# Jan-Celin/SCCG-genome-compression

Hardware: AMD Instinct MI355X
Metric: target bases compressed/sec at 1/2/4/8 GPUs; bit-exact record stream vs CPU ref (higher is better)
Workload: dtype u8

## Files before the change

### sccg-genome-compression_amd/csrc/ingest.hip

```cpp
#include "internal.h"

namespace {

constexpr int PER_T = INGEST_TILE / SCCG_BLOCK;
constexpr int WPB = SCCG_BLOCK / 64;


constexpr int64_t FM_CHUNK = 16384;
template <int NW>
__device__ __forceinline__ uint8_t wb(const uint32_t (&w)[NW], int i) { return (uint8_t)(w[i >> 2] >> (8 * (i & 3))); }
template <int NW>
__device__ __forceinline__ void load_words(const uint8_t* __restrict__ buf, int64_t n, int64_t off, uint32_t (&w)[NW]);
__global__ __launch_bounds__(SCCG_BLOCK) void k_first_match(const uint8_t* __restrict__ buf, int64_t n,
                                                            const int64_t* __restrict__ from_slot, int mode, uint8_t c,
                                                            int64_t* __restrict__ res, unsigned int* __restrict__ ticket) {
    __shared__ int64_t s_cs;
    const int64_t from = from_slot ? *from_slot + 1 : 0;
    const int64_t base = from & ~(int64_t)63;
    constexpr int PER = FM_CHUNK / SCCG_BLOCK;
    for (;;) {
        if (threadIdx.x == 0) {
            const int64_t cs = base + (int64_t)atomicAdd(ticket, 1u) * FM_CHUNK;
            const int64_t best = (int64_t)__hip_atomic_load((unsigned long long*)res, __ATOMIC_RELAXED, __HIP_MEMORY_SCOPE_AGENT);
            s_cs = (cs >= n || cs >= best) ? -1 : cs;
// ... 663 lines not shown
            if (q >= 0 && t - q > RUNS_LOOKBACK) atomicOr(ovf, 2);
            const uint32_t first = (uint32_t)(f >> 1) & 3u;
#pragma unroll
            for (int p = 0; p < 2; p++) {
                const uint32_t fp = (first >> p) & 1u, pp = (prev >> p) & 1u;
                if (fp && !pp) b |= 1 << (2 * p);
                if (!fp && pp) b |= 2 << (2 * p);
            }
        }
        bev[t] = b;
        cs[t] = (int64_t)((c & 0xffff) + (b & 1)) | ((int64_t)(((c >> 32) & 0xffff) + ((b >> 2) & 1)) << 32);
        ce[t] = (int64_t)(((c >> 16) & 0xffff) + ((b >> 1) & 1)) | ((int64_t)((c >> 48) + ((b >> 3) & 1)) << 32);
    }
}

__global__ void k_runs_copy(int64_t ntiles, const int64_t* __restrict__ toff, const uint64_t* __restrict__ rc,
                            const int32_t* __restrict__ bev, const int64_t* __restrict__ cs, const int64_t* __restrict__ ce,
                            RunSlots rsl, int32_t* __restrict__ rs_l, int32_t* __restrict__ re_l,
                            int32_t* __restrict__ rs_n, int32_t* __restrict__ re_n) {
    for (int64_t t = (int64_t)blockIdx.x * blockDim.x + threadIdx.x; t < ntiles; t += (int64_t)gridDim.x * blockDim.x) {
        const uint64_t c = rc[t];
        const int32_t b = bev[t];
        const int32_t t0 = (int32_t)toff[t];
        const size_t sb = (size_t)t * RUN_SLOT;
        int32_t* const dst[4] = {rs_l, re_l, rs_n, re_n};
        const int32_t* const src[4] = {rsl.sl, rsl.el, rsl.sn, rsl.en};
        const int64_t base[4] = {cs[t] & 0xffffffff, ce[t] & 0xffffffff, cs[t] >> 32, ce[t] >> 32};
#pragma unroll
        for (int q = 0; q < 4; q++) {
            const int end = q & 1;
            int64_t at = base[q];
            if ((b >> q) & 1) dst[q][at++] = t0 - end;
            const int nq = (int)((c >> (16 * q)) & 0xffff);
            for (int k = 0; k < nq && k < RUN_SLOT; k++) dst[q][at++] = src[q][sb + k] - end;
        }
    }
}

__global__ void k_runs_fin(const int64_t* __restrict__ tot, const int64_t* __restrict__ d_nT, int32_t* __restrict__ re_l,
                           int32_t* __restrict__ re_n, int64_t* __restrict__ d_nruns) {
    const int64_t sl = tot[0] & 0xffffffff, sn = tot[0] >> 32, el = tot[1] & 0xffffffff, en = tot[1] >> 32;
    if (sl > el) re_l[sl - 1] = (int32_t)(*d_nT - 1);
    if (sn > en) re_n[sn - 1] = (int32_t)(*d_nT - 1);
    d_nruns[0] = sl;
    d_nruns[1] = sn;
}

__device__ __forceinline__ int64_t run_text_len(int32_t d, int32_t len, bool at_end) {
    return len == 1 ? (int64_t)ndigits_i32(d) + (at_end ? 0 : 1) : (int64_t)(3 + ndigits_i32(d) + ndigits_i32(len));
}

__global__ void k_run_textlen(const int32_t* __restrict__ rs, const int32_t* __restrict__ re, int64_t nr,
                              int64_t n, int64_t* __restrict__ len) {
    for (int64_t r = (int64_t)blockIdx.x * blockDim.x + threadIdx.x; r < nr; r += (int64_t)gridDim.x * blockDim.x) {
        const int32_t d = rs[r] - (r ? rs[r - 1] : 0);
        len[r] = run_text_len(d, re[r] - rs[r] + 1, (int64_t)re[r] == n - 1);
    }
}

__global__ void k_run_textwrite(const int32_t* __restrict__ rs, const int32_t* __restrict__ re, int64_t nr,
                                int64_t n, const int64_t* __restrict__ off, uint8_t* __restrict__ out) {
    for (int64_t r = (int64_t)blockIdx.x * blockDim.x + threadIdx.x; r < nr; r += (int64_t)gridDim.x * blockDim.x) {
        const int32_t d = rs[r] - (r ? rs[r - 1] : 0);
        const int32_t len = re[r] - rs[r] + 1;
        uint8_t* o = out + off[r];
        if (len == 1) {
            o += write_i32(o, d);
            if ((int64_t)re[r] != n - 1) *o = ',';
        } else {
            *o++ = '(';
            o += write_i32(o, d);
            *o++ = ',';
            o += write_i32(o, len);
            *o = ')';
        }
    }
}

}

constexpr int FH_T = 256, FH_PER = 64;
__global__ __launch_bounds__(FH_T) void k_find_header(const uint8_t* __restrict__ buf, int64_t n, int64_t* __restrict__ d_sc,
                                                      int32_t* __restrict__ ovf) {
    __shared__ unsigned long long s_hit;
    int64_t res[2] = {n, n};
    for (int ph = 0; ph < 2; ph++) {
        if (ph == 1 && res[0] >= n) break;
        const int64_t from = ph == 0 ? 0 : res[0] + 1;
        for (int64_t cs = from & ~(int64_t)63; cs < n; cs += (int64_t)FH_T * FH_PER) {
            if (threadIdx.x == 0) s_hit = ~0ull;
            __syncthreads();
            const int64_t p0 = cs + (int64_t)threadIdx.x * FH_PER;
            if (p0 < n) {
                uint32_t w[FH_PER / 4];
                load_words<FH_PER / 4>(buf, n, p0, w);
                uint8_t prev = p0 > 0 ? buf[p0 - 1] : (uint8_t)'\n';
                int64_t hit = -1;
#pragma unroll
                for (int i = 0; i < FH_PER; i++) {
                    const uint8_t c = wb(w, i);
                    const int64_t p = p0 + i;
                    const bool ok = p >= from && p < n && (ph == 0 ? (c == '>' && prev == '\n') : c == '\n');
                    if (ok && hit < 0) hit = p;
                    prev = c;
                }
                if (hit >= 0) atomicMin(&s_hit, (unsigned long long)hit);
            }
            __syncthreads();
            const unsigned long long h = s_hit;
            __syncthreads();
            if (h != ~0ull) { res[ph] = (int64_t)h; break; }
        }
    }
    if (threadIdx.x == 0) {
        d_sc[0] = res[0]; d_sc[1] = res[1]; d_sc[2] = 0; d_sc[3] = 0;
        d_sc[20] = (int64_t)INT32_MAX << 32;
        d_sc[21] = (int64_t)INT32_MAX;
        *reinterpret_cast<int32_t*>(d_sc + 32) = 0;
        if (ovf) *ovf = 0;
    }
}

int launch_first_match(const uint8_t* buf, int64_t n, const int64_t* from_slot, int mode, uint8_t c, int64_t* res,
                       int64_t* ticket_slot, hipStream_t s) {
    int rc = dev_set_i64(res, 1, {n}, s);
    if (!rc) rc = dev_set_i64(ticket_slot, 1, {0}, s);
    if (rc) return rc;
    if (n > 0) {
        hipLaunchKernelGGL(k_first_match, dim3(64), dim3(SCCG_BLOCK), 0, s, buf, n, from_slot, mode, c, res,
                           reinterpret_cast<unsigned int*>(ticket_slot));
        SCCG_HIP(hipGetLastError());
    }
    return 0;
}

int launch_find_header(const uint8_t* buf, int64_t n, int64_t* d_sc, int32_t* d_ovf, hipStream_t s) {
    hipLaunchKernelGGL(k_find_header, dim3(1), dim3(FH_T), 0, s, buf, n, d_sc, d_ovf);
    SCCG_HIP(hipGetLastError());
    return 0;
}

int launch_fasta_strip(IngestMode mode, const uint8_t* buf, int64_t n, const int64_t* d_header, uint8_t* out,
                       int64_t* d_len, int32_t* d_flags, const IngestScratch& sc, hipStream_t s, FilterMode fmode,
                       uint8_t* out2, int64_t* d_len2, const RunSlots* runs) {
    if (n <= 0) {
        SCCG_HIP(hipMemsetAsync(d_len, 0, sizeof(int64_t), s));
        if (d_len2) SCCG_HIP(hipMemsetAsync(d_len2, 0, sizeof(int64_t), s));
        return 0;
    }
    if (!out2) fmode = FILTER_UPPER;
    const int64_t ntiles = (n + STRIP_TILE - 1) / STRIP_TILE;
    const unsigned g = grid_for(ntiles, WPB);
    uint16_t* const kc = sc.keep_cache;
    int32_t* const kf = sc.keep_flag;
#define SUMMARY(M, K)                                                                                                   \
    hipLaunchKernelGGL((k_strip_summary<M, K>), dim3(g), dim3(SCCG_BLOCK), 0, s, fmode, buf, n, d_header, sc.tile_a,   \
                       sc.tile_b, sc.tile_fa, sc.tile_fb, sc.tile_last, kc, kf)
    if (mode == INGEST_TGT && kc) SUMMARY(INGEST_TGT, true);
    else if (mode == INGEST_TGT) SUMMARY(INGEST_TGT, false);
    else if (kc) SUMMARY(INGEST_REF, true);
    else SUMMARY(INGEST_REF, false);
#undef SUMMARY
    const int64_t nblk = (ntiles + SCAN_B - 1) / SCAN_B;
    if (nblk > SCAN_B) return SCCG_E_UNSUPPORTED;
    TileSum* btot = reinterpret_cast<TileSum*>(sc.block_sums);
    hipLaunchKernelGGL(k_strip_scan, dim3((unsigned)nblk), dim3(SCAN_T), 0, s, ntiles, sc.tile_a, sc.tile_b, sc.tile_fa,
                       sc.tile_fb, sc.tile_last, btot, sc.scan_ticket, d_len, d_len2);
    const StripScan sp{sc.tile_a, sc.tile_b, sc.tile_fa, sc.tile_fb, sc.tile_last, btot};
    const RunSlots rsl = runs ? *runs : RunSlots{};
    if (mode == INGEST_TGT && runs)
        PROF_LAUNCH(PROF_STRIP, s, (k_strip_write<INGEST_TGT, true>), dim3(g), dim3(SCCG_BLOCK), 0, s, fmode, buf, n, d_header, sp,
                    sc.tile_off, sc.tile_off2, sc.tile_carry, out, out2, d_flags, rsl, (const uint16_t*)kc, (const int32_t*)kf);
    else if (mode == INGEST_TGT)
        PROF_LAUNCH(PROF_STRIP, s, (k_strip_write<INGEST_TGT, false>), dim3(g), dim3(SCCG_BLOCK), 0, s, fmode, buf, n, d_header, sp,
                    sc.tile_off, sc.tile_off2, sc.tile_carry, out, out2, d_flags, rsl, (const uint16_t*)kc, (const int32_t*)kf);
    else
        PROF_LAUNCH(PROF_STRIP, s, (k_strip_write<INGEST_REF, false>), dim3(g), dim3(SCCG_BLOCK), 0, s, fmode, buf, n, d_header, sp,
                    sc.tile_off, sc.tile_off2, sc.tile_carry, out, out2, d_flags, rsl, (const uint16_t*)kc, (const int32_t*)kf);
    SCCG_HIP(hipGetLastError());
    return 0;
}

int launch_runs2(const uint8_t* in, int64_t n, int32_t* rs_l, int32_t* re_l, int32_t* rs_n, int32_t* re_n,
                 int64_t* d_nruns, int64_t* d_cnt_l, int64_t* d_cnt_n, int64_t* d_partial, hipStream_t s) {
    if (n <= 0) {
        SCCG_HIP(hipMemsetAsync(d_nruns, 0, 2 * sizeof(int64_t), s));
        return 0;
    }
    const int64_t ntiles = (n + INGEST_TILE - 1) / INGEST_TILE;
    hipLaunchKernelGGL(k_runs_count, dim3((unsigned)ntiles), dim3(SCCG_BLOCK), 0, s, in, n, d_cnt_l, d_cnt_n);
    int rc = dev_excl_sum(d_cnt_l, d_cnt_l, ntiles, d_nruns, d_partial, s);
    if (!rc) rc = dev_excl_sum(d_cnt_n, d_cnt_n, ntiles, d_nruns + 1, d_partial, s);
    if (rc) return rc;
    PROF_LAUNCH(PROF_RUNS, s, k_runs_write, dim3((unsigned)ntiles), dim3(SCCG_BLOCK), 0, s, in, n,
// ... 66 lines not shown
```

### sccg-genome-compression_amd/csrc/scan.hip

```cpp
#include "internal.h"

#include <cstring>

namespace {

constexpr int ITEMS = 16;
constexpr int TILE = SCCG_BLOCK * ITEMS;

struct OpSum {
    static __device__ __forceinline__ int64_t id() { return 0; }
    static __device__ __forceinline__ int64_t f(int64_t a, int64_t b) { return a + b; }
};
struct OpMax {
    static __device__ __forceinline__ int64_t id() { return INT64_MIN; }
    static __device__ __forceinline__ int64_t f(int64_t a, int64_t b) { return a > b ? a : b; }
};

template <class Op>
__device__ __forceinline__ int64_t wave_incl(int64_t v) {
    const int lane = lane_id();
#pragma unroll
    for (int d = 1; d < 64; d <<= 1) {
        int64_t o = __shfl_up(v, d, 64);
        if (lane >= d) v = Op::f(v, o);
// ... 191 lines not shown
__global__ void k_put_framed(uint8_t* __restrict__ dst, const uint8_t* __restrict__ src, int64_t n, uint8_t pre,
                             uint8_t post) {
    for (int64_t i = (int64_t)blockIdx.x * blockDim.x + threadIdx.x; i < n + 2; i += (int64_t)gridDim.x * blockDim.x)
        dst[i] = i == 0 ? pre : (i == n + 1 ? post : src[i - 1]);
}
}

int dev_put_framed(uint8_t* dst, const uint8_t* src, int64_t n, char pre, char post, hipStream_t s) {
    const unsigned g = grid_for(n + 2, 256) > 1024 ? 1024 : grid_for(n + 2, 256);
    hipLaunchKernelGGL(k_put_framed, dim3(g), dim3(256), 0, s, dst, src, n, (uint8_t)pre, (uint8_t)post);
    SCCG_HIP(hipGetLastError());
    return 0;
}

namespace {
__global__ void k_put_frame(uint8_t* __restrict__ out, const uint8_t* __restrict__ hdr, int64_t hlen, int64_t total) {
    for (int64_t i = (int64_t)blockIdx.x * blockDim.x + threadIdx.x; i <= hlen; i += (int64_t)gridDim.x * blockDim.x)
        out[i] = i < hlen ? hdr[i] : (uint8_t)'\n';
    if (blockIdx.x == 0 && threadIdx.x == 0) out[total - 1] = '\n';
}
}

int dev_put_frame(uint8_t* out, const uint8_t* hdr, int64_t hlen, int64_t total, hipStream_t s) {
    const unsigned g = grid_for(hlen + 1, 256) > 64 ? 64 : grid_for(hlen + 1, 256);
    hipLaunchKernelGGL(k_put_frame, dim3(g), dim3(256), 0, s, out, hdr, hlen, total);
    SCCG_HIP(hipGetLastError());
    return 0;
}

int dev_put_bytes(uint8_t* p, const char* bytes, int n, hipStream_t s) {
    Bytes16 v{};
    if (n > 16) return SCCG_E_INTERNAL;
    for (int i = 0; i < n; i++) v.v[i] = (uint8_t)bytes[i];
    hipLaunchKernelGGL(k_set_u8, dim3(1), dim3(64), 0, s, p, n, v);
    SCCG_HIP(hipGetLastError());
    return 0;
}

int dev_set_i64(int64_t* p, int n, std::initializer_list<int64_t> vals, hipStream_t s) {
    Vals8 v{};
    int i = 0;
    for (int64_t x : vals) if (i < 8) v.v[i++] = x;
    hipLaunchKernelGGL(k_set_i64, dim3(1), dim3(64), 0, s, p, n < i ? n : i, v);
    SCCG_HIP(hipGetLastError());
    return 0;
}
int dev_set_i32(int32_t* p, int n, std::initializer_list<int32_t> vals, hipStream_t s) {
    Vals8i v{};
    int i = 0;
    for (int32_t x : vals) if (i < 8) v.v[i++] = x;
    hipLaunchKernelGGL(k_set_i32, dim3(1), dim3(64), 0, s, p, n < i ? n : i, v);
    SCCG_HIP(hipGetLastError());
    return 0;
}

int64_t scan_partials_needed(int64_t n) { return (n + TILE - 1) / TILE + 1; }

int dev_excl_sum(const int64_t* in, int64_t* out, int64_t n, int64_t* d_total, int64_t* d_partial,
                 hipStream_t s) {
    return scan_one<OpSum>(in, out, n, d_total, d_partial, s);
}

int dev_excl_sum2(const int64_t* in0, int64_t* out0, int64_t* d_total0, const int64_t* in1, int64_t* out1,
                  int64_t* d_total1, int64_t n, int64_t* d_partial, hipStream_t s) {
    const int64_t np = scan_partials_needed(n);
    const ScanArrays a{{in0, in1}, {out0, out1}, {d_total0, d_total1}, {d_partial, d_partial + np}};
    return scan_impl<OpSum>(a, 2, n, s);
}

int dev_excl_max(const int64_t* in, int64_t* out, int64_t n, int64_t* d_total, int64_t* d_partial,
                 hipStream_t s) {
    return scan_one<OpMax>(in, out, n, d_total, d_partial, s);
}

namespace {
constexpr int RB_MAX = 8;
constexpr int RB_BYTES = 4096 - 64;
struct RbArgs {
    const uint8_t* src[RB_MAX];
    int32_t off[RB_MAX];
    int32_t bytes[RB_MAX];
    int32_t n;
};
__global__ void k_readback(RbArgs a, uint8_t* __restrict__ host, unsigned long long* flag, unsigned long long seq) {
    for (int i = 0; i < a.n; i++) {
        const uint8_t* src = a.src[i];
        uint8_t* dst = host + a.off[i];
        const int nb = a.bytes[i];
        if ((((uintptr_t)src) & 3) == 0 && (nb & 3) == 0) {
            for (int b = (int)threadIdx.x; b < nb / 4; b += (int)blockDim.x)
                reinterpret_cast<uint32_t*>(dst)[b] = reinterpret_cast<const uint32_t*>(src)[b];
        } else {
            for (int b = (int)threadIdx.x; b < nb; b += (int)blockDim.x) dst[b] = src[b];
        }
    }
    __threadfence_system();
    __syncthreads();
    if (threadIdx.x == 0) __hip_atomic_store(flag, seq, __ATOMIC_RELEASE, __HIP_MEMORY_SCOPE_SYSTEM);
}
struct RbHost {
    uint8_t* buf = nullptr;
    uint8_t* dbuf = nullptr;
    unsigned long long seq = 0;
};
thread_local RbHost g_rb;
}

int dev_readback(const RbItem* items, int n, hipStream_t s) {
    if (n <= 0) return 0;
    if (n > RB_MAX) return SCCG_E_INVALID;
    if (!g_rb.buf) {
        void* p = nullptr;
        SCCG_HIP(hipHostMalloc(&p, 4096, hipHostMallocMapped | hipHostMallocCoherent | hipHostMallocPortable));
        void* dp = nullptr;
        SCCG_HIP(hipHostGetDevicePointer(&dp, p, 0));
        g_rb.buf = static_cast<uint8_t*>(p);
        g_rb.dbuf = static_cast<uint8_t*>(dp);
        *reinterpret_cast<volatile unsigned long long*>(g_rb.buf) = 0;
    }
    RbArgs a{};
    int off = 0;
    for (int i = 0; i < n; i++) {
        if (items[i].bytes < 0 || off + items[i].bytes > RB_BYTES) return SCCG_E_INVALID;
        a.src[i] = static_cast<const uint8_t*>(items[i].src);
        a.off[i] = off;
        a.bytes[i] = items[i].bytes;
        off += (items[i].bytes + 7) & ~7;
    }
    a.n = n;
    const unsigned long long seq = ++g_rb.seq;
    unsigned long long* flag = reinterpret_cast<unsigned long long*>(g_rb.buf);
    hipLaunchKernelGGL(k_readback, dim3(1), dim3(64), 0, s, a, g_rb.dbuf + 64,
                       reinterpret_cast<unsigned long long*>(g_rb.dbuf), seq);
    SCCG_HIP(hipGetLastError());
    for (uint64_t it = 1;; it++) {
        if (__atomic_load_n(flag, __ATOMIC_ACQUIRE) == seq) break;
        if ((it & 4095) == 0) {
            const hipError_t e = hipStreamQuery(s);
            if (e != hipErrorNotReady) {
                SCCG_HIP(e == hipSuccess ? hipStreamSynchronize(s) : e);
                if (__atomic_load_n(flag, __ATOMIC_ACQUIRE) != seq) {
                    return sccg_hip_fail(hipErrorUnknown, "readback flag not raised by a finished stream", __FILE__,
                                         __LINE__);
                }
                break;
            }
        }
        __builtin_ia32_pause();
    }
    for (int i = 0; i < n; i++) memcpy(items[i].dst, g_rb.buf + 64 + a.off[i], (size_t)items[i].bytes);
    return 0;
}
```

### sccg-genome-compression_amd/csrc/walk.hip

```cpp
#include "internal.h"

#include <algorithm>
#include <chrono>
#include <map>
#include <mutex>
#include <cstdio>
#include <cstdlib>
#include <vector>

namespace {

constexpr int WPB = 4;
constexpr int WWPB = 4;
constexpr int WCAP = 256;
constexpr int32_t INVALID = INT32_MIN;
constexpr int32_t NEVER = INT32_MIN + 1;
constexpr int ANCHOR_K = 32;
constexpr int KEY_K = 15;
constexpr int KMAX = 32;
constexpr int KB_COUNT = 32;
constexpr int ANCHOR_STEP = 64;
constexpr int ANCHOR_LOAD = 1;
constexpr int ANCHOR_PROBE_BATCHES = 2;
constexpr uint32_t A_MULTI = 0xFFFFFFFFu;
// ... 101 lines not shown
    int32_t* chm_t;
    int32_t* chm_p;
    int32_t* chm_l;
    int32_t chm_cap;
    int32_t ch_settled;
    int32_t* chh_y;
    uint32_t* chh_k;
    int32_t* chh_n;
    int32_t* chh_tr;
    uint64_t* dbg;
    int32_t dbg_phases;
    int32_t dbg_round;
};

__device__ __forceinline__ int32_t chunk_lo(const WalkPtrs& A, int32_t j) { return A.xlo + j * A.S; }
__device__ __forceinline__ int32_t chunk_hi(const WalkPtrs& A, int32_t j) {
    const int32_t lo = A.xlo + j * A.S;
    return lo + A.S < A.xhi ? lo + A.S : A.xhi;
}

constexpr int WFBITS = 14;
constexpr int LBV = 2048;
constexpr int LBW = LBV / 256;
static_assert(LBW % 8 == 0, "whole 32-byte stretches per lane");
constexpr int LEAD = 128;
static_assert(LEAD % (4 * LBW) == 0, "the lead is whole lanes' stretches");
__device__ __forceinline__ uint32_t wf_h1(uint32_t key) { return slot_hash(key, WFBITS); }
__device__ __forceinline__ uint32_t wf_h2(uint32_t key) { return (key * 0x85EBCA77u) >> (32 - WFBITS); }
__device__ __forceinline__ uint32_t wf_h3(uint32_t key) { return (key * 0xC2B2AE3Du + 0x27D4EB2Fu) >> (32 - WFBITS); }
struct WalkLds {
    uint32_t wbits[1 << (WFBITS - 5)];
    __attribute__((aligned(16))) uint8_t rbuf[LBV + 64];
    __attribute__((aligned(16))) uint8_t tbuf[LBV + 64];
};
constexpr int32_t NO_BUF = INT32_MIN / 2;
struct BufPos {
    int32_t rb0 = NO_BUF, tb0 = NO_BUF;
    __device__ __forceinline__ bool has_r(int32_t a, int32_t n) const { return a >= rb0 && a + n <= rb0 + LBV; }
    __device__ __forceinline__ bool has_t(int32_t a, int32_t n) const { return a >= tb0 && a + n <= tb0 + LBV; }
};

__device__ __forceinline__ uint64_t pick_key(int32_t p, int32_t pme) {
    const int32_t d = p - pme;
    return ((uint64_t)(uint32_t)(d < 0 ? -d : d) << 32) | (uint32_t)p;
}

__device__ __forceinline__ bool bytes_eq(const uint8_t* a, const uint8_t* b, int k) {
    for (int i = 0; i < k; i++) if (a[i] != b[i]) return false;
    return true;
}

template <int ND>
__device__ __forceinline__ void loadw_lds(const uint8_t* lds, int32_t off, uint32_t (&o)[ND]) {
    const uint32_t* w = reinterpret_cast<const uint32_t*>(lds) + (off >> 2);
    const uint32_t sh = (uint32_t)(off & 3);
    uint32_t v[ND + 1];
#pragma unroll
    for (int i = 0; i <= ND; i++) v[i] = w[i];
#pragma unroll
    for (int i = 0; i < ND; i++) o[i] = __builtin_amdgcn_alignbyte(v[i + 1], v[i], sh);
}

template <int ND>
__device__ __forceinline__ void loadw_sel(bool in_lds, const uint8_t* lds, int32_t lds_off, const uint8_t* g,
                                          uint32_t (&o)[ND]) {
    if (in_lds) {
        loadw_lds<ND>(lds, lds_off, o);
    } else {
        loadw<ND>(g, o);
        asm volatile("" ::: "memory");
    }
}

template <int N>
__device__ __forceinline__ int first_diff(const uint32_t (&r)[N], const uint32_t (&t)[N]) {
    int pos = 4 * N;
#pragma unroll
    for (int i = N - 1; i >= 0; i--) {
        const uint32_t x = r[i] ^ t[i];
        if (x) pos = 4 * i + (__builtin_ctz(x) >> 3);
    }
    return pos;
}
__device__ __forceinline__ int first_diff32(const uint32_t (&r)[8], const uint32_t (&t)[8]) { return first_diff<8>(r, t); }

__device__ __forceinline__ void lds16(const uint8_t* lds, int32_t off, uint32_t (&o)[4]) {
    const int32_t a = off + 16 * lane_id();
    const uint2* p = reinterpret_cast<const uint2*>(lds + (a & ~7));
    const uint2 v0 = p[0], v1 = p[1], v2 = p[2];
    const uint32_t sh = (uint32_t)(off & 3);
    uint32_t w[5];
    if (off & 4) { w[0] = v0.y; w[1] = v1.x; w[2] = v1.y; w[3] = v2.x; w[4] = v2.y; }
    else { w[0] = v0.x; w[1] = v0.y; w[2] = v1.x; w[3] = v1.y; w[4] = v2.x; }
#pragma unroll
    for (int i = 0; i < 4; i++) o[i] = __builtin_amdgcn_alignbyte(w[i + 1], w[i], sh);
}

__device__ __forceinline__ int32_t lds_first_diff(const uint8_t* rbuf, int32_t ra, const uint8_t* tbuf, int32_t tb, int32_t n) {
    const int lane = lane_id();
    for (int32_t base = 0; base < n; base += 1024) {
        const int32_t lim = n - base - 16 * lane;
        int e = 16;
        if (lim > 0) {
            uint32_t r[4], t[4];
            lds16(rbuf, ra + base, r);
            lds16(tbuf, tb + base, t);
            e = first_diff<4>(r, t);
            if (e >= lim) e = 16;
        }
        const unsigned long long m = __ballot(e < 16);
        if (m) {
            const int l = first_lane(m);
            return base + 16 * l + lane_val(e, l);
        }
    }
    return n;
}

__device__ __forceinline__ int32_t wave_lce(const WalkPtrs& A, WalkLds& L, BufPos& B, int32_t a, int32_t b, int32_t maxlen) {
    const int lane = lane_id();
    if (maxlen <= 0) return 0;
    int32_t off = 0;
    if (a >= B.rb0 && b >= B.tb0 && a < B.rb0 + LBV && b < B.tb0 + LBV) {
        int32_t avail = B.rb0 + LBV - a < B.tb0 + LBV - b ? B.rb0 + LBV - a : B.tb0 + LBV - b;
        if (avail > maxlen) avail = maxlen;
        const int32_t e = lds_first_diff(L.rbuf, a - B.rb0, L.tbuf, b - B.tb0, avail);
        if (e < avail || avail >= maxlen) return e;
        off = avail;
    }
    while (off < maxlen) {
        const int32_t lead = (a + off >= LEAD && b + off >= LEAD) ? LEAD : 0;
        const int32_t sa = (a + off - lead) & ~15, sb = (b + off - lead) & ~15;
        static_assert(LBV == 2048, "two KiB of each per step");
        const uint4* gr = reinterpret_cast<const uint4*>(A.R + sa) + lane;
        const uint4* gt = reinterpret_cast<const uint4*>(A.T + sb) + lane;
        const uint4 r0 = gr[0], r1 = gr[64], t0 = gt[0], t1 = gt[64];
        wave_sync();
        {
            uint4* dr = reinterpret_cast<uint4*>(L.rbuf) + lane;
            uint4* dt = reinterpret_cast<uint4*>(L.tbuf) + lane;
            dr[0] = r0; dr[64] = r1;
            dt[0] = t0; dt[64] = t1;
        }
        wave_sync();
        B.rb0 = sa;
        B.tb0 = sb;
        const int32_t ra = a + off - sa, tb = b + off - sb;
        int32_t avail = LBV - (ra > tb ? ra : tb);
        if (avail > maxlen - off) avail = maxlen - off;
        const int32_t e = lds_first_diff(L.rbuf, ra, L.tbuf, tb, avail);
        if (e < avail) return off + e;
        off += avail;
    }
    return maxlen;
}


__device__ int32_t wave_lce_hbm(const uint8_t* __restrict__ R, int32_t a, const uint8_t* __restrict__ T, int32_t b,
                                int32_t maxlen) {
    const int lane = lane_id();
    for (int32_t off = 0; off < maxlen; off += 2048) {
        const int32_t my = off + 32 * lane;
        int32_t e = INT32_MAX;
        if (maxlen - my > 0) {
            uint32_t r[8], t[8];
            loadw<8>(R + a + my, r);
            loadw<8>(T + b + my, t);
            int pos = first_diff32(r, t);
            if (maxlen - my < 32 && pos > maxlen - my) pos = maxlen - my;
            if (pos < 32) e = my + pos;
        }
        const unsigned long long sm = __ballot(e != INT32_MAX);
        if (sm) {
            const int32_t m = lane_val(e, first_lane(sm));
            return m < maxlen ? m : maxlen;
        }
    }
    return maxlen > 0 ? maxlen : 0;
}

__device__ __forceinline__ int32_t ext_k(const WalkPtrs& A, WalkLds& L, BufPos& B, int32_t c, int32_t y) {
    const int32_t kp = A.kp;
    int32_t maxlen = A.nR - (c + kp);
    const int32_t mt = A.nT - (y + kp);
    if (mt < maxlen) maxlen = mt;
    const int32_t l = kp + wave_lce(A, L, B, c + kp, y + kp, maxlen);
    return l >= A.k ? l : 0;
}

constexpr uint32_t KEY_NONE = 0x40000000u;
struct RegWin {
    int32_t P, lo, n;
    uint32_t key[4];
    uint32_t vmask;
};

__device__ __forceinline__ void reg_window(const WalkPtrs& A, int32_t P, RegWin& W, const WalkLds* L = nullptr,
                                           const BufPos* B = nullptr) {
    const int lane = lane_id(), k = A.k;
    W.P = P;
    W.lo = P - A.m < 0 ? 0 : P - A.m;
    const int32_t hi = (P + A.m < A.nR - k) ? P + A.m : A.nR - k;
    W.n = hi - W.lo + 1;
    if (W.n < 0) W.n = 0;
    W.vmask = 0;
    W.key[0] = W.key[1] = W.key[2] = W.key[3] = KEY_NONE;
    const bool lds = L && B->has_r(W.lo, W.n + 20);
    const int i0 = 4 * lane;
    if (i0 >= W.n) return;
    uint32_t w[5];
    loadw_sel<5>(lds, lds ? L->rbuf : nullptr, lds ? W.lo - B->rb0 + i0 : 0, A.R + W.lo + i0, w);
    uint64_t code;
    uint32_t bad;
    pack_codes<5>(w, code, bad);
    const int kp = A.kp;
    const uint32_t MASK = (1u << (2 * kp)) - 1u, KM = (1u << kp) - 1u;
#pragma unroll
    for (int q = 0; q < 4; q++) {
        W.key[q] = (bad >> q) & KM ? exotic_key(A.R + W.lo + i0 + q, kp) : (uint32_t)(code >> (2 * q)) & MASK;
        if (i0 + q < W.n) W.vmask |= 1u << q;
        else W.key[q] = KEY_NONE;
    }
}

__device__ __forceinline__ uint32_t target_key_w(const WalkPtrs& A, int32_t y, const uint32_t (&w)[4]) {
    const int kp = A.kp;
    uint64_t code;
    uint32_t bad;
    pack_codes<4>(w, code, bad);
    return bad & ((1u << kp) - 1u) ? exotic_key(A.T + y, kp) : (uint32_t)code & ((1u << (2 * kp)) - 1u);
}

__device__ __forceinline__ uint32_t win_match(const WalkPtrs& A, const RegWin& W, uint32_t kk, int32_t y) {
    uint32_t m = 0;
#pragma unroll
    for (int q = 0; q < 4; q++)
        if (((W.vmask >> q) & 1u) && W.key[q] == kk) m |= 1u << q;
    if (m && kk >= KEY_EXOTIC) {
        const int32_t c0 = W.lo + 4 * lane_id();
        for (int q = 0; q < 4; q++)
            if (((m >> q) & 1u) && !bytes_eq(A.R + c0 + q, A.T + y, A.kp)) m &= ~(1u << q);
    }
    return m;
}

__device__ __forceinline__ bool win_any(const RegWin& W, uint32_t kk) {
    return (W.key[0] == kk) | (W.key[1] == kk) | (W.key[2] == kk) | (W.key[3] == kk);
}

__device__ void bloom_window(const RegWin& W, WalkLds& L) {
    const int lane = lane_id();
    uint4* b4 = reinterpret_cast<uint4*>(L.wbits);
    for (int i = lane; i < (1 << (WFBITS - 5)) / 4; i += 64) b4[i] = make_uint4(0, 0, 0, 0);
// ... 425 lines not shown
        if (!(A.conv[j] || !pred_changed)) continue;
        A.cur[j] = 1 - A.cur[j];
        A.exitX[j] = A.newX[j];
        A.exitP[j] = A.newP[j];
        A.usedX[j] = A.snapX[j];
        A.usedP[j] = A.snapP[j];
        A.seedq[j] = 0;
        if (A.frozen[j]) {
            A.flist[atomicAdd(&A.scal[5], 1)] = j;
            atomicOr(&A.fbits[j >> 5], 1u << (j & 31));
        }
    }
    if (!grid_last_block(reinterpret_cast<unsigned int*>(A.scal + 14), &last)) return;
    sort_list_block(A, A.flist, A.scal + 5, A.fbits, wsum);
}

__device__ __forceinline__ void sort_list_block(const WalkPtrs& A, int32_t* __restrict__ list, const int32_t* __restrict__ count,
                                                uint32_t* __restrict__ bits, int32_t* wsum) {
    if (*count <= 0) return;
    const int32_t nw = (A.C + 31) >> 5;
    const int32_t per = (nw + LS_T - 1) / LS_T, w0 = (int32_t)threadIdx.x * per;
    const int32_t w1 = w0 + per < nw ? w0 + per : nw;
    int c = 0;
    for (int32_t w = w0; w < w1; w++) c += __popc(bits[w]);
    const int incl = wave_incl_add<int>(c);
    const int wv = (int)(threadIdx.x >> 6), lane = lane_id();
    if (lane == 63) wsum[wv] = incl;
    __syncthreads();
    if (threadIdx.x == 0) {
        int run = 0;
        for (int i = 0; i < LS_T / 64; i++) { const int x = wsum[i]; wsum[i] = run; run += x; }
    }
    __syncthreads();
    int at = wsum[wv] + incl - c;
    for (int32_t w = w0; w < w1; w++) {
        uint32_t b = bits[w];
        if (!b) continue;
        bits[w] = 0;
        for (; b; b &= b - 1) list[at++] = (w << 5) + __ffs((int)b) - 1;
    }
}
__global__ __launch_bounds__(LS_T) void k_list_sort(WalkPtrs A, int32_t* __restrict__ list, const int32_t* __restrict__ count,
                                                    uint32_t* __restrict__ bits) {
    __shared__ int32_t wsum[LS_T / 64 + 1];
    if (A.scal[9]) return;
    sort_list_block(A, list, count, bits, wsum);
}

constexpr unsigned FZ_GRID = 256;
constexpr int FZ_T = SCCG_BLOCK;
__global__ __launch_bounds__(SCCG_BLOCK) void k_frozen_scan(WalkPtrs A, int fbase) {
    __shared__ WalkLds lds_all[WPB];
    if (A.scal[9]) return;
    const int fi = (int)blockIdx.y, f = fbase + fi;
    if (f >= A.scal[5]) return;
    const int32_t j = A.flist[f];
    const int32_t x0 = A.exitX[j], P = A.exitP[j];
    WalkLds& L = lds_all[wave_in_block()];
    RegWin W;
    reg_window(A, P, W);
    if (W.n <= 0) return;
    bloom_window(W, L);
    const int32_t end = A.nT - A.k + 1 < A.xhi ? A.nT - A.k + 1 : A.xhi;
    const int64_t gw = (int64_t)blockIdx.x * WPB + wave_in_block(), G = (int64_t)gridDim.x * WPB;
    for (int64_t base = x0 + gw * 64 * WIDE; base < end; base += G * 64 * WIDE) {
        if (base >= (int64_t)__hip_atomic_load(&A.fy[fi], __ATOMIC_RELAXED, __HIP_MEMORY_SCOPE_AGENT)) return;
        const int32_t seg_end = base + 64 * WIDE < end ? (int32_t)(base + 64 * WIDE) : end;
        const int32_t y = wide_scan(A, L, W, (int32_t)base, seg_end);
        if (y < seg_end) {
            if (lane_id() == 0) atomicMin(&A.fy[fi], y);
            return;
        }
    }
}

__device__ __forceinline__ int32_t fill_last(const WalkPtrs& A, int32_t j, int32_t y) {
    const int32_t lastk1 = A.nT - A.k + 1;
    const int32_t cap = A.xhi < lastk1 ? A.xhi : lastk1;
    if (y >= cap) return A.C - 1;
    if (y < A.xlo) return j;
    const int32_t q = (y - A.xlo) / A.S - 1;
    return q < j ? j : (q > A.C - 1 ? A.C - 1 : q);
}
template <bool DEV>
__global__ void k_walk_init(WalkPtrs A, int32_t startX, int32_t startP) {
    if (DEV && blockIdx.x == 0 && threadIdx.x == 0) {
        const unsigned long long* r = A.fc + 4;
        if (r[8] != 2 && r[0] == 0 && r[4] > 0) {
            const uint64_t k0 = 1ull << 32;
            const uint64_t pk = (r[5] >= 2 && r[6]) ? r[7] : ((r[6] && k0 < r[7]) ? k0 : r[7]);
            startX = (int32_t)r[4];
            startP = (int32_t)(uint32_t)pk + (int32_t)r[4] - 1;
        } else {
            startX = A.nT - A.k + 1;
            startP = INVALID;
        }
    }
    if (blockIdx.x == 0 && threadIdx.x == 0) A.scal[9] = DEV && startP == INVALID ? 1 : 0;
    for (int32_t j = (int32_t)(blockIdx.x * blockDim.x + threadIdx.x); j < A.C; j += (int32_t)(gridDim.x * blockDim.x)) {
        A.cur[j] = 0;
        A.cnt[0][j] = 0;
        A.cnt[1][j] = 0;
        A.usedX[j] = NEVER;
        A.usedP[j] = NEVER;
        A.exitX[j] = INVALID;
        A.exitP[j] = INVALID;
        A.kind[j] = j ? KIND_SPEC : KIND_FIX;
        A.plist[j] = j;
        A.lround[j] = 1;
        A.seedq[j] = 0;
        A.trapped[j] = 0;
        A.tflag[j] = 0;
        A.hintY[j] = -1;
        A.walked[j] = 0;
        A.changed[j] = 0;
        A.conv[j] = 0;
        A.frozen[j] = 0;
    }
    for (int32_t w = (int32_t)(blockIdx.x * blockDim.x + threadIdx.x); w <= A.C / 32; w += (int32_t)(gridDim.x * blockDim.x)) {
        A.fbits[w] = 0;
        A.cbits[w] = 0;
    }
    if (blockIdx.x == 0 && threadIdx.x == 0) {
        A.scal[0] = 0; A.scal[1] = 0; A.scal[2] = startX; A.scal[3] = startP;
        A.scal[5] = 0;
        A.scal[11] = 0;
        A.scal[14] = 0; A.scal[15] = 0;
        A.snapX[0] = startX;
        A.snapP[0] = startP;
    }
}

__global__ void k_spec_rest(WalkPtrs A) {
    const int32_t next = A.round + 1;
    for (int32_t q = (int32_t)(blockIdx.x * blockDim.x + threadIdx.x); q < A.C; q += (int32_t)(gridDim.x * blockDim.x)) {
        if (A.usedX[q] != NEVER || A.lround[q] == next) continue;
        A.kind[q] = KIND_SPEC;
        A.lround[q] = next;
        A.plist[atomicAdd(&A.scal[0], 1)] = q;
    }
}

__global__ __launch_bounds__(FROZEN_MAX) void k_round_fill(WalkPtrs A, int fbase, int fcap) {
    if (A.scal[9]) return;
    __shared__ int32_t rj[FROZEN_MAX], ry[FROZEN_MAX], sj[FROZEN_MAX], sy[FROZEN_MAX];
    const int t = (int)threadIdx.x;
    int nf = fcap > 0 ? A.scal[5] - fbase : 0;
    if (nf > fcap) nf = fcap;
    if (nf < 0) nf = 0;
    int32_t j = 0, y = 0;
    if (t < nf) { j = A.flist[fbase + t]; y = A.fy[t]; rj[t] = j; ry[t] = y; }
    __syncthreads();
    if (t < nf) {
        int r = 0;
        for (int f = 0; f < nf; f++) r += rj[f] < j || (rj[f] == j && f < t);
        sj[r] = j;
        sy[r] = y;
    }
    __syncthreads();
    if (t == 0) {
        int na = 0;
        int32_t filled_to = -1;
        for (int r = 0; r < nf; r++) {
            const int32_t jr = sj[r];
            if (jr <= filled_to || jr + 1 >= A.C) continue;
            const int32_t last = fill_last(A, jr, sy[r]);
            if (last > jr) { A.fa_j[na] = jr; A.fa_l[na] = last; A.fa_p[na] = A.exitP[jr]; na++; }
            if (last + 1 < A.C && sy[r] != INT32_MAX) { A.hintY[last + 1] = sy[r]; A.hintP[last + 1] = A.exitP[jr]; }
            filled_to = last;
        }
        A.scal[13] = na;
        A.scal[0] = 0;
        A.scal[12] = 0;
    }
}

constexpr int RT_T = 256;
__global__ __launch_bounds__(RT_T) void k_round_close(WalkPtrs A) {
    if (A.scal[9]) return;
    __shared__ int32_t fj[FROZEN_MAX], fl[FROZEN_MAX], fp[FROZEN_MAX];
    __shared__ int32_t trig[RESPEC_MAX_TRIGGERS];
    __shared__ int32_t wsum[RT_T / 64 + 1];
    __shared__ int last;
    const int na = A.scal[13];
    for (int i = (int)threadIdx.x; i < na; i += RT_T) { fj[i] = A.fa_j[i]; fl[i] = A.fa_l[i]; fp[i] = A.fa_p[i]; }
    __syncthreads();
    const int32_t next = A.round + 1;
    const int32_t lastk1 = A.nT - A.k + 1;
    auto filled = [&](int32_t q, int32_t* P) -> bool {
        int lo = 0, hi = na;
        while (lo < hi) {
            const int mid = (lo + hi) >> 1;
            if (fj[mid] < q) lo = mid + 1; else hi = mid;
        }
        if (lo == 0 || q > fl[lo - 1]) return false;
        *P = fp[lo - 1];
        return true;
    };
    const int32_t j = (int32_t)(blockIdx.x * blockDim.x + threadIdx.x);
    if (j < A.C) {
        int32_t ux, up, P = 0;
        if (na && filled(j, &P)) {
            const int32_t lo_j = chunk_lo(A, j), hi_j = chunk_hi(A, j);
            ux = lo_j < lastk1 ? lo_j : lastk1;
// ... 737 lines not shown
}

__global__ __launch_bounds__(SCCG_BLOCK) void k_first_kmer(const uint8_t* __restrict__ fa, int64_t n,
                                                           const int64_t* __restrict__ hdr, int k, int64_t limit,
                                                           uint8_t* __restrict__ kb) {
    __shared__ int64_t tmp[5];
    constexpr int PER = 64;
    const int64_t h = hdr[0], he = hdr[1];
    const int64_t end = n < limit ? n : limit;
    int64_t found = 0;
    for (int64_t base = 0; base < end && found < k; base += (int64_t)SCCG_BLOCK * PER) {
        const int64_t p0 = base + (int64_t)threadIdx.x * PER;
        uint32_t w[PER / 4];
        if (p0 + PER + 4 <= end) {
            loadw<PER / 4>(fa + p0, w);
        } else {
#pragma unroll
            for (int q = 0; q < PER / 4; q++) {
                uint32_t v = 0;
                for (int i = 0; i < 4; i++) {
                    const int64_t p = p0 + 4 * q + i;
                    v |= (uint32_t)(p < end ? fa[p] : (uint8_t)' ') << (8 * i);
                }
                w[q] = v;
            }
        }
        uint64_t keep = 0;
#pragma unroll
        for (int i = 0; i < PER; i++) {
            const uint8_t b = (uint8_t)(w[i >> 2] >> (8 * (i & 3)));
            const int64_t p = p0 + i;
            const bool kp = p < end && !(p >= h && p < he) && !c_isspace(b) && c_toupper(b) != 'N';
            keep |= (uint64_t)kp << i;
        }
        int64_t total = 0;
        int64_t idx = found + block_excl_add((int64_t)__popcll(keep), tmp, &total);
        for (uint64_t m = keep; m && idx < k; m &= m - 1, idx++) {
            const int i = __ffsll((long long)m) - 1;
            kb[idx] = c_toupper((uint8_t)(w[i >> 2] >> (8 * (i & 3))));
        }
        found += total;
    }
    if (threadIdx.x == 0) *reinterpret_cast<int32_t*>(kb + KB_COUNT) = found < k ? (int32_t)found : k;
}

__global__ __launch_bounds__(SCCG_BLOCK) void k_sweep_early(WalkPtrs A) {
    const int k = A.k, kp = A.kp;
    const int64_t nR = A.dnR ? *A.dnR : A.nR;
    const bool have = *reinterpret_cast<const int32_t*>(A.kb + KB_COUNT) == k;
    const uint32_t key0 = have ? walk_key(A.kb, kp) : KEY_EXOTIC;
    const bool want = key0 < KEY_EXOTIC;
    sweep_kmers_w(A.R, nR - k + 1, kp, [&](uint32_t code, bool pure) { return want && pure && code == key0; },
                  [&](int64_t c) {
                      if (k > kp && !bytes_eq(A.R + c + kp, A.kb + kp, k - kp)) return;
                      const unsigned long long i = atomicAdd(&A.fc[13], 1ull);
                      if (i < (unsigned long long)CAND_CAP) A.cand[i] = (int32_t)c;
                  },
                  [&](int64_t p0, const uint32_t (&cw)[20], const uint32_t (&dw)[20], uint32_t acc) {
                      anchor_samples(A, nR, p0, cw, dw, acc);
                  });
}

constexpr int CAND_STATS_GRID = 256;
__device__ __forceinline__ bool cand_stats_usable(const WalkPtrs& A) {
    const int k = A.k, lane = lane_id();
    const bool head = *reinterpret_cast<const int32_t*>(A.kb + KB_COUNT) == k && A.fc[13] <= (unsigned long long)CAND_CAP &&
                      A.nT >= k;
    const bool same = lane >= k || A.kb[lane] == A.T[lane];
    return head && __ballot(!same) == 0 && walk_key(A.kb, A.kp) < KEY_EXOTIC;
}
__global__ __launch_bounds__(SCCG_BLOCK) void k_cand_stats(WalkPtrs A) {
    __shared__ CandBest wbest[SCCG_BLOCK / 64];
    __shared__ int ok, last;
    const int k = A.k;
    const unsigned long long cnt = A.fc[13];
    if (threadIdx.x < 64) {
        const bool u = cand_stats_usable(A);
        if (threadIdx.x == 0) ok = u;
    }
    __syncthreads();
    CandBest v{0, 0, 0, ~0ull};
    if (ok) {
        const unsigned long long nw = (unsigned long long)gridDim.x * (SCCG_BLOCK / 64);
        for (unsigned long long i = blockIdx.x * (SCCG_BLOCK / 64) + (threadIdx.x >> 6); i < cnt; i += nw) {
            const int32_t c = A.cand[i];
            int32_t maxlen = A.nR - (c + k);
            if (A.nT - k < maxlen) maxlen = A.nT - k;
            const uint32_t l = (uint32_t)(k + wave_lce_hbm(A.R, c + k, A.T, k, maxlen));
            v = cb_merge(v, CandBest{l, 1u, c == 0 ? 1u : 0u, c ? pick_key(c, -1) : ~0ull});
        }
    }
    if (lane_id() != 0) v = CandBest{0, 0, 0, ~0ull};
    v = cb_wave(v);
    if (lane_id() == 0) wbest[threadIdx.x >> 6] = v;
    __syncthreads();
    if (threadIdx.x == 0) {
        for (int i = 1; i < SCCG_BLOCK / 64; i++) v = cb_merge(v, wbest[i]);
        unsigned long long* o = A.fcb + 4 * blockIdx.x;
        o[0] = v.l; o[1] = v.cnt; o[2] = v.has0; o[3] = v.minkey;
    }
    if (!grid_last_block(reinterpret_cast<unsigned int*>(A.fc + 14), &last)) return;
    if (threadIdx.x == 0) A.fc[12] = ok ? 1 : 2;
    if (!ok) return;
    v = CandBest{0, 0, 0, ~0ull};
    for (int b = (int)threadIdx.x; b < (int)gridDim.x; b += SCCG_BLOCK) {
        const unsigned long long* o = A.fcb + 4 * b;
        v = cb_merge(v, CandBest{(uint32_t)o[0], (uint32_t)o[1], (uint32_t)o[2], o[3]});
    }
    v = cb_wave(v);
    if (lane_id() == 0) wbest[threadIdx.x >> 6] = v;
    __syncthreads();
    if (threadIdx.x == 0) {
        for (int i = 1; i < SCCG_BLOCK / 64; i++) v = cb_merge(v, wbest[i]);
        A.fc[8] = v.l; A.fc[9] = v.cnt; A.fc[10] = v.has0; A.fc[11] = v.minkey;
        A.fc[4] = v.cnt ? 0ull : ~0ull;
        A.fc[5] = ~0ull;
    }
}

__global__ __launch_bounds__(1024) void k_cand_reduce(WalkPtrs A, int nblk, int32_t x0) {
    __shared__ CandBest wbest[16];
    CandBest v{0, 0, 0, ~0ull};
    for (int b = (int)threadIdx.x; b < nblk; b += (int)blockDim.x) {
        const unsigned long long* o = A.fcb + 4 * b;
        v = cb_merge(v, CandBest{(uint32_t)o[0], (uint32_t)o[1], (uint32_t)o[2], o[3]});
    }
    v = cb_wave(v);
    if (lane_id() == 0) wbest[threadIdx.x >> 6] = v;
    __syncthreads();
    if (threadIdx.x == 0) {
        for (int i = 1; i < (int)(blockDim.x >> 6); i++) v = cb_merge(v, wbest[i]);
        A.fc[8] = v.l; A.fc[9] = v.cnt; A.fc[10] = v.has0; A.fc[11] = v.minkey;
        if (x0 >= 0) { A.fc[4] = v.cnt ? (unsigned long long)x0 : ~0ull; A.fc[5] = ~0ull; A.fc[12] = 0; }
    }
}

__global__ void k_chunk_counts(WalkPtrs A) {
    for (int32_t j = (int32_t)(blockIdx.x * blockDim.x + threadIdx.x); j < A.C; j += (int32_t)(gridDim.x * blockDim.x))
        A.flat_off[j] = A.cnt[A.cur[j]][j];
}

__global__ __launch_bounds__(SCCG_BLOCK) void k_flatten(WalkPtrs A, int32_t first) {
    const int32_t j = (int32_t)blockIdx.x * WPB + wave_in_block();
    if (j >= A.C) return;
    const int lane = lane_id();
    const int32_t b = A.cur[j];
    const int32_t n = A.cnt[b][j];
    const int64_t o = A.flat_off[j] + first;
    const int32_t* t = A.bt[b] + (size_t)j * A.cap;
    const int32_t* p = A.bp[b] + (size_t)j * A.cap;
    const int32_t* l = A.bl[b] + (size_t)j * A.cap;
    for (int i = lane; i < n; i += 64) { A.ft[o + i] = t[i]; A.fp[o + i] = p[i]; A.fl[o + i] = l[i]; }
}

constexpr int64_t LONG_PIECE = 64 * 1024;
__device__ __forceinline__ void queue_long(const WalkPtrs& A, int64_t src, int64_t dst, int64_t len) {
    const int64_t np = (len + LONG_PIECE - 1) / LONG_PIECE;
    const int64_t e = (int64_t)atomicAdd((unsigned long long*)&A.scal64[2], (unsigned long long)np);
    for (int64_t i = 0; i < np && e + i < A.lgap_cap; i++) {
        int64_t* q = A.lgap + 3 * (e + i);
        q[0] = src + i * LONG_PIECE;
        q[1] = dst + i * LONG_PIECE;
        q[2] = len - i * LONG_PIECE < LONG_PIECE ? len - i * LONG_PIECE : LONG_PIECE;
    }
}

__device__ __forceinline__ void wave_copy(const uint8_t* __restrict__ s, uint8_t* __restrict__ d, int64_t n) {
// ... 1251 lines not shown
```

Baseline: 188.6 billion.

## Vectorize header scan, shrink LCE stride, add launch bounds and scalar hints

```diff
diff --git a/sccg-genome-compression_amd/csrc/ingest.hip b/sccg-genome-compression_amd/csrc/ingest.hip
--- a/sccg-genome-compression_amd/csrc/ingest.hip
+++ b/sccg-genome-compression_amd/csrc/ingest.hip
@@ -769,34 +769,54 @@
 constexpr int FH_T = 256, FH_PER = 64;
 __global__ __launch_bounds__(FH_T) void k_find_header(const uint8_t* __restrict__ buf, int64_t n, int64_t* __restrict__ d_sc,
                                                       int32_t* __restrict__ ovf) {
-    __shared__ unsigned long long s_hit;
+    __shared__ unsigned int s_hit;
+    constexpr int NW = FH_PER / 4;
     int64_t res[2] = {n, n};
     for (int ph = 0; ph < 2; ph++) {
         if (ph == 1 && res[0] >= n) break;
         const int64_t from = ph == 0 ? 0 : res[0] + 1;
         for (int64_t cs = from & ~(int64_t)63; cs < n; cs += (int64_t)FH_T * FH_PER) {
-            if (threadIdx.x == 0) s_hit = ~0ull;
+            if (threadIdx.x == 0) s_hit = ~0u;
             __syncthreads();
             const int64_t p0 = cs + (int64_t)threadIdx.x * FH_PER;
             if (p0 < n) {
-                uint32_t w[FH_PER / 4];
-                load_words<FH_PER / 4>(buf, n, p0, w);
-                uint8_t prev = p0 > 0 ? buf[p0 - 1] : (uint8_t)'\n';
-                int64_t hit = -1;
-#pragma unroll
-                for (int i = 0; i < FH_PER; i++) {
-                    const uint8_t c = wb(w, i);
-                    const int64_t p = p0 + i;
-                    const bool ok = p >= from && p < n && (ph == 0 ? (c == '>' && prev == '\n') : c == '\n');
-                    if (ok && hit < 0) hit = p;
-                    prev = c;
+                const int skip = from > p0 ? (int)(from - p0 < FH_PER ? from - p0 : FH_PER) : 0;
+                const uint8_t prev = p0 > 0 ? buf[p0 - 1] : (uint8_t)'\n';
+                int hit = -1;
+                if (p0 + FH_PER <= n && (((uintptr_t)(buf + p0)) & 15) == 0) {
+                    const uint4* src = reinterpret_cast<const uint4*>(buf + p0);
+                    uint32_t w[NW];
+#pragma unroll
+                    for (int q = 0; q < NW / 4; q++) {
+                        const uint4 v = src[q];
+                        w[4 * q] = v.x; w[4 * q + 1] = v.y; w[4 * q + 2] = v.z; w[4 * q + 3] = v.w;
+                    }
+                    uint32_t carry = prev == '\n' ? 0x80000000u : 0u;
+                    uint64_t hm = 0;
+#pragma unroll
+                    for (int q = 0; q < NW; q++) {
+                        const uint32_t nl = sw_eq(w[q], '\n');
+                        const uint32_t m = ph == 0 ? sw_eq(w[q], '>') & ((nl << 8) | (carry >> 24)) : nl;
+                        carry = nl;
+                        hm |= (uint64_t)sw_bits(m) << (4 * q);
+                    }
+                    hm = skip < FH_PER ? hm & (~0ull << skip) : 0;
+                    if (hm) hit = __ffsll((long long)hm) - 1;
+                } else {
+                    uint8_t pv = prev;
+#pragma unroll 1
+                    for (int i = 0; i < FH_PER && p0 + i < n; i++) {
+                        const uint8_t c = buf[p0 + i];
+                        if (i >= skip && (ph == 0 ? (c == '>' && pv == '\n') : c == '\n')) { hit = i; break; }
+                        pv = c;
+                    }
                 }
-                if (hit >= 0) atomicMin(&s_hit, (unsigned long long)hit);
+                if (hit >= 0) atomicMin(&s_hit, threadIdx.x * FH_PER + (unsigned int)hit);
             }
             __syncthreads();
-            const unsigned long long h = s_hit;
+            const unsigned int h = s_hit;
             __syncthreads();
-            if (h != ~0ull) { res[ph] = (int64_t)h; break; }
+            if (h != ~0u) { res[ph] = cs + (int64_t)h; break; }
         }
     }
     if (threadIdx.x == 0) {
diff --git a/sccg-genome-compression_amd/csrc/scan.hip b/sccg-genome-compression_amd/csrc/scan.hip
--- a/sccg-genome-compression_amd/csrc/scan.hip
+++ b/sccg-genome-compression_amd/csrc/scan.hip
@@ -297,7 +297,7 @@
     int32_t bytes[RB_MAX];
     int32_t n;
 };
-__global__ void k_readback(RbArgs a, uint8_t* __restrict__ host, unsigned long long* flag, unsigned long long seq) {
+__global__ __launch_bounds__(64) void k_readback(RbArgs a, uint8_t* __restrict__ host, unsigned long long* flag, unsigned long long seq) {
     for (int i = 0; i < a.n; i++) {
         const uint8_t* src = a.src[i];
         uint8_t* dst = host + a.off[i];
diff --git a/sccg-genome-compression_amd/csrc/walk.hip b/sccg-genome-compression_amd/csrc/walk.hip
--- a/sccg-genome-compression_amd/csrc/walk.hip
+++ b/sccg-genome-compression_amd/csrc/walk.hip
@@ -207,7 +207,6 @@
     }
     return pos;
 }
-__device__ __forceinline__ int first_diff32(const uint32_t (&r)[8], const uint32_t (&t)[8]) { return first_diff<8>(r, t); }
 
 __device__ __forceinline__ void lds16(const uint8_t* lds, int32_t off, uint32_t (&o)[4]) {
     const int32_t a = off + 16 * lane_id();
@@ -283,17 +282,18 @@
 
 __device__ int32_t wave_lce_hbm(const uint8_t* __restrict__ R, int32_t a, const uint8_t* __restrict__ T, int32_t b,
                                 int32_t maxlen) {
+    constexpr int ND = 4, NB = 4 * ND;
     const int lane = lane_id();
-    for (int32_t off = 0; off < maxlen; off += 2048) {
-        const int32_t my = off + 32 * lane;
+    for (int32_t off = 0; off < maxlen; off += 64 * NB) {
+        const int32_t my = off + NB * lane;
         int32_t e = INT32_MAX;
         if (maxlen - my > 0) {
-            uint32_t r[8], t[8];
-            loadw<8>(R + a + my, r);
-            loadw<8>(T + b + my, t);
-            int pos = first_diff32(r, t);
-            if (maxlen - my < 32 && pos > maxlen - my) pos = maxlen - my;
-            if (pos < 32) e = my + pos;
+            uint32_t r[ND], t[ND];
+            loadw<ND>(R + a + my, r);
+            loadw<ND>(T + b + my, t);
+            int pos = first_diff<ND>(r, t);
+            if (maxlen - my < NB && pos > maxlen - my) pos = maxlen - my;
+            if (pos < NB) e = my + pos;
         }
         const unsigned long long sm = __ballot(e != INT32_MAX);
         if (sm) {
@@ -885,8 +885,13 @@
     const int32_t q = (y - A.xlo) / A.S - 1;
     return q < j ? j : (q > A.C - 1 ? A.C - 1 : q);
 }
+template <typename T, typename V>
+__device__ __forceinline__ void put32(T* p, uint32_t j, V v) {
+    static_assert(sizeof(T) == 4, "dword arrays");
+    *reinterpret_cast<T*>(reinterpret_cast<char*>(p) + (j << 2)) = (T)v;
+}
 template <bool DEV>
-__global__ void k_walk_init(WalkPtrs A, int32_t startX, int32_t startP) {
+__global__ __launch_bounds__(256) void k_walk_init(WalkPtrs A, int32_t startX, int32_t startP) {
     if (DEV && blockIdx.x == 0 && threadIdx.x == 0) {
         const unsigned long long* r = A.fc + 4;
         if (r[8] != 2 && r[0] == 0 && r[4] > 0) {
@@ -900,29 +905,30 @@
         }
     }
     if (blockIdx.x == 0 && threadIdx.x == 0) A.scal[9] = DEV && startP == INVALID ? 1 : 0;
-    for (int32_t j = (int32_t)(blockIdx.x * blockDim.x + threadIdx.x); j < A.C; j += (int32_t)(gridDim.x * blockDim.x)) {
-        A.cur[j] = 0;
-        A.cnt[0][j] = 0;
-        A.cnt[1][j] = 0;
-        A.usedX[j] = NEVER;
-        A.usedP[j] = NEVER;
-        A.exitX[j] = INVALID;
-        A.exitP[j] = INVALID;
-        A.kind[j] = j ? KIND_SPEC : KIND_FIX;
-        A.plist[j] = j;
-        A.lround[j] = 1;
-        A.seedq[j] = 0;
-        A.trapped[j] = 0;
-        A.tflag[j] = 0;
-        A.hintY[j] = -1;
-        A.walked[j] = 0;
-        A.changed[j] = 0;
-        A.conv[j] = 0;
-        A.frozen[j] = 0;
-    }
-    for (int32_t w = (int32_t)(blockIdx.x * blockDim.x + threadIdx.x); w <= A.C / 32; w += (int32_t)(gridDim.x * blockDim.x)) {
-        A.fbits[w] = 0;
-        A.cbits[w] = 0;
+    const uint32_t nC = (uint32_t)A.C, step = gridDim.x * blockDim.x;
+    for (uint32_t j = blockIdx.x * blockDim.x + threadIdx.x; j < nC; j += step) {
+        put32(A.cur, j, 0);
+        put32(A.cnt[0], j, 0);
+        put32(A.cnt[1], j, 0);
+        put32(A.usedX, j, NEVER);
+        put32(A.usedP, j, NEVER);
+        put32(A.exitX, j, INVALID);
+        put32(A.exitP, j, INVALID);
+        put32(A.kind, j, j ? KIND_SPEC : KIND_FIX);
+        put32(A.plist, j, j);
+        put32(A.lround, j, 1);
+        put32(A.seedq, j, 0);
+        put32(A.trapped, j, 0);
+        put32(A.tflag, j, 0);
+        put32(A.hintY, j, -1);
+        put32(A.walked, j, 0);
+        put32(A.changed, j, 0);
+        put32(A.conv, j, 0);
+        put32(A.frozen, j, 0);
+    }
+    for (uint32_t w = blockIdx.x * blockDim.x + threadIdx.x; w <= nC / 32; w += step) {
+        put32(A.fbits, w, 0);
+        put32(A.cbits, w, 0);
     }
     if (blockIdx.x == 0 && threadIdx.x == 0) {
         A.scal[0] = 0; A.scal[1] = 0; A.scal[2] = startX; A.scal[3] = startP;
@@ -1826,7 +1832,8 @@
     CandBest v{0, 0, 0, ~0ull};
     if (ok) {
         const unsigned long long nw = (unsigned long long)gridDim.x * (SCCG_BLOCK / 64);
-        for (unsigned long long i = blockIdx.x * (SCCG_BLOCK / 64) + (threadIdx.x >> 6); i < cnt; i += nw) {
+        const unsigned wv = (unsigned)__builtin_amdgcn_readfirstlane((int)(threadIdx.x >> 6));
+        for (unsigned long long i = blockIdx.x * (SCCG_BLOCK / 64) + wv; i < cnt; i += nw) {
             const int32_t c = A.cand[i];
             int32_t maxlen = A.nR - (c + k);
             if (A.nT - k < maxlen) maxlen = A.nT - k;
```

Result: no change. 189.0 billion (median of 4 runs) (+0.2%).
